# hendraet/synthesis-in-style

Hardware: AMD Instinct MI355X
Metric: StyleGAN2 synth images/sec + seg-train images/sec @256², 1/2/4/8 MI355X (higher is better)
Workload: dtype f32; 1 GPU; StyleGAN2 Generator(256,512,8,cm=2).forward, batch 32 per GPU, explicit noise, return_intermediate_activations=True (BASELINE.json configs[1]); batch_per_gpu=32, image_size=256, parallelism=replicated x1, images sharded, no collective

## Files before the change

### synthesis-in-style_amd/csrc/modconv_upfir.hip

```cpp
#include <type_traits>
#include "modconv_common.h"

namespace {

constexpr int UF_MBLK = 64;
constexpr int UF_PLANES = 16;
constexpr int UF_WROW = UF_PLANES * UF_MBLK + 32;
constexpr int UF_XP_MAX = 4;
constexpr unsigned UF_OOB = 0x80000000u;

struct UpFirParams {
    const float* x; const float* u; const float* s; const float* dscale; float* out;
    int B, Cin, Cout, H, W, OH, ORS;
    int nbw, bps, total_blocks;
    int vr;
    int rw4;
    int xs;
};

template <int PIPE, int ABL = 0, int NW = 8>
__global__ __launch_bounds__(64 * NW) __attribute__((amdgpu_waves_per_eu(2, 2))) void modconv_upfir_kernel(const UpFirParams p) {
    constexpr int UF_CC = NW, UF_NBLK = 8 * NW, UF_THREADS = 64 * NW;
    extern __shared__ __attribute__((aligned(16))) float lds[];
    float* Wl = lds;
    float* Xl = Wl + 2 * UF_CC * UF_WROW;
    float* Sl = Xl + 2 * UF_CC * p.xs;
    const int tid = threadIdx.x, lane = tid & 63, wave = __builtin_amdgcn_readfirstlane(tid >> 6);
    const int l15 = lane & 15, kq = lane >> 4;
    const int wm = wave & 1, wn = wave >> 1;

    const int n_co = p.Cout / UF_MBLK;
    const int tile = blockIdx.x / n_co, o0 = (blockIdx.x % n_co) * UF_MBLK;
    const int g0 = tile * UF_NBLK;
    const int b_first = g0 / p.bps, bh_first = (g0 % p.bps) / p.nbw;
    const int R0 = b_first * p.vr + 2 * bh_first;
    const int RW = 4 * p.rw4;
    const int HW = p.H * p.W;

    const int g = g0 + wn * 16 + l15;
    const bool live = g < p.total_blocks;
    const int gc = live ? g : p.total_blocks - 1;
    const int b = gc / p.bps, rem = gc % p.bps, bh = rem / p.nbw, bw = rem % p.nbw;
    const int xoff = (b * p.vr + 2 * bh - R0) * RW + 3 + 2 * bw;
    const int soff = (b - b_first) * p.Cin;

    for (int e = tid; e < 2 * p.Cin; e += UF_THREADS) {
        const int n = e / p.Cin, ci = e - n * p.Cin;
        Sl[e] = p.s[(int64_t)min(b_first + n, p.B - 1) * p.Cin + ci];
    }

    const __amdgpu_buffer_rsrc_t w_rsrc = sis_buffer_rsrc(p.u + 2 * o0);
    const __amdgpu_buffer_rsrc_t x_rsrc = sis_buffer_rsrc(p.x);
    const unsigned w_voff = (unsigned)(((lane >> 5) * p.Cout * 2 + (lane & 31) * 4) * 4);
    const int xpieces = p.xs >> 8;
    unsigned x_voff[UF_XP_MAX];
#pragma unroll
    for (int q = 0; q < UF_XP_MAX; ++q) {
        const int i = q * 64 + lane;
        const int row = i / p.rw4, c4 = i - row * p.rw4;
        const int v = R0 + row;
        const int bb = v / p.vr, h = v - bb * p.vr - 1, col = 4 * (c4 - 1);
        const bool ok = q < xpieces && bb < p.B && h >= 0 && h < p.H && col >= 0 && col < p.W;
        x_voff[q] = ok ? (unsigned)((bb * p.Cin * HW + h * p.W + col) * 4) : UF_OOB;
    }
    auto stage = [&](int ci0, int buf) {
        float* wdst = Wl + (buf * UF_CC + wave) * UF_WROW;
        const unsigned wbase = (unsigned)((ci0 + wave) * UF_PLANES * p.Cout * 4);
#pragma unroll
        for (int q = 0; q < 4; ++q) sis_buffer_load_lds16(w_rsrc, wdst + q * 256, w_voff, wbase + (unsigned)(q * 2 * p.Cout * 2 * 4));
        float* xdst = Xl + (buf * UF_CC + wave) * p.xs;
        const unsigned xbase = (unsigned)((ci0 + wave) * HW * 4);
#pragma unroll
        for (int q = 0; q < UF_XP_MAX; ++q)
            if (q < xpieces) sis_buffer_load_lds16(x_rsrc, xdst + q * 256, x_voff[q], xbase);
    };

    sis_f32x4 acc[5][5][2];
#pragma unroll
    for (int a = 0; a < 5; ++a)
#pragma unroll
        for (int c = 0; c < 5; ++c)
#pragma unroll
            for (int t = 0; t < 2; ++t) acc[a][c][t] = sis_f32x4{0.f, 0.f, 0.f, 0.f};

    __syncthreads();
    stage(0, 0);
    __syncthreads();

    if constexpr (PIPE == 4) {
        static_assert(NW == 4 && ABL == 0, "pipelined form: 4-wave workgroups, no ablations");
        const int n_chunks = p.Cin / UF_CC;
        if (n_chunks > 1) stage(UF_CC, 1);
        __syncthreads();
        float tA[4][4], tB[4][4], cm0[4], raw[3][3], svn;
        auto tr_read = [&](int c, int bufc) {
            const int cl = min(c, n_chunks - 1) * UF_CC + kq;
            svn = Sl[soff + cl];
            const float* xb = Xl + (bufc * UF_CC + kq) * p.xs + xoff;
#pragma unroll
            for (int r = 0; r < 3; ++r)
#pragma unroll
                for (int j = 0; j < 3; ++j) raw[r][j] = xb[r * RW + j];
        };
        auto tr_col = [&](int r, float (&t)[4][4]) {
            const float d0 = raw[r][0] * svn, d1 = raw[r][1] * svn, d2 = raw[r][2] * svn;
            float* o = r == 0 ? cm0 : (r == 1 ? t[1] : t[3]);
            o[0] = d0 - d1; o[1] = d1; o[2] = d2 - d1; o[3] = d2;
            asm volatile("" : "+v"(o[0]), "+v"(o[1]), "+v"(o[2]), "+v"(o[3]));
        };
        auto tr_row = [&](float (&t)[4][4]) {
#pragma unroll
            for (int j = 0; j < 4; ++j) {
                t[0][j] = cm0[j] - t[1][j]; t[2][j] = t[3][j] - t[1][j];
                asm volatile("" : "+v"(t[0][j]), "+v"(t[2][j]));
            }
        };
        tr_read(0, 0);
#pragma unroll
        for (int r = 0; r < 3; ++r) tr_col(r, tA);
        tr_row(tA);
        const int woff = kq * UF_WROW + (wm * 32 + l15) * 2;
        sis_f32x2 ra[3][2];
        ra[0][0] = *reinterpret_cast<const sis_f32x2*>(Wl + woff); ra[0][1] = *reinterpret_cast<const sis_f32x2*>(Wl + woff + 32);
        auto chunk = [&](auto parity, int c, const float (&t)[4][4], float (&tn)[4][4]) {
            constexpr int B = decltype(parity)::value;
            const float* wb = Wl + B * UF_CC * UF_WROW + woff;
            auto fetch = [&](int k) {
                ra[k % 3][0] = *reinterpret_cast<const sis_f32x2*>(wb + k * 2 * UF_MBLK);
                ra[k % 3][1] = *reinterpret_cast<const sis_f32x2*>(wb + k * 2 * UF_MBLK + 32);
            };
            fetch(1);
#pragma unroll
            for (int k = 0; k < 8; ++k) {
                if (k + 2 < 8) fetch(k + 2);
                if (k == 7) {
                    ra[0][0] = *reinterpret_cast<const sis_f32x2*>(Wl + (B ^ 1) * UF_CC * UF_WROW + woff);
                    ra[0][1] = *reinterpret_cast<const sis_f32x2*>(Wl + (B ^ 1) * UF_CC * UF_WROW + woff + 32);
                }
#pragma unroll
                for (int e = 0; e < 2; ++e) {
                    const int i = 2 * k + e, u = i >> 2, v = i & 3;
                    const float a0 = ra[k % 3][0][e], a1 = ra[k % 3][1][e];
#pragma unroll
                    for (int pp = 0; pp < 2; ++pp)
#pragma unroll
                        for (int qq = 0; qq < 2; ++qq) {
                            if ((pp && u != 3) || (qq && v != 3)) continue;
                            const int pi = u + pp, qi = v + qq;
                            const int di = pi == 3 ? 1 : (pi == 4 ? 3 : pi), dj = qi == 3 ? 1 : (qi == 4 ? 3 : qi);
                            acc[pi][qi][0] = __builtin_amdgcn_mfma_f32_16x16x4f32(a0, t[di][dj], acc[pi][qi][0], 0, 0, 0);
                            acc[pi][qi][1] = __builtin_amdgcn_mfma_f32_16x16x4f32(a1, t[di][dj], acc[pi][qi][1], 0, 0, 0);
                        }
                    if (k >= 5) {
                        if (k == 5 && e == 1) {
                            asm volatile("s_waitcnt vmcnt(0)" ::: "memory");
                            __syncthreads();
                            if (c + 2 < n_chunks) stage((c + 2) * UF_CC, B);
                            tr_read(c + 1, B ^ 1);
                        }
                        if (k == 6 && e == 0) { tr_col(0, tn); tr_col(1, tn); }
                        if (k == 6 && e == 1) tr_col(2, tn);
                        if (k == 7 && e == 0) tr_row(tn);
                        __builtin_amdgcn_sched_barrier(0);
                    }
                }
                if (k < 5) {
                    if (k + 2 < 8) __builtin_amdgcn_sched_group_barrier(0x100, 1, 0);
                    const int u = (2 * k) >> 2, vhi = ((2 * k) & 3) + 1;
                    if (u == 3 && vhi == 3) __builtin_amdgcn_sched_group_barrier(0x008, 12, 0);
                    else if (u == 3) __builtin_amdgcn_sched_group_barrier(0x008, 8, 0);
                    else if (vhi == 3) __builtin_amdgcn_sched_group_barrier(0x008, 6, 0);
                    else __builtin_amdgcn_sched_group_barrier(0x008, 4, 0);
                }
            }
        };
        for (int c = 0; c < n_chunks; c += 2) {
            chunk(std::integral_constant<int, 0>(), c, tA, tB);
            if (c + 1 < n_chunks) chunk(std::integral_constant<int, 1>(), c + 1, tB, tA);
        }
    } else {
    int buf = 0;
    float t0[4][4] = {}, t1[4][4] = {};
    const bool late_dma = PIPE == 3 && wave >= 4;
    for (int ci0 = 0; ci0 < p.Cin; ci0 += UF_CC, buf ^= 1) {
        if (!(ABL & 2) && !late_dma && ci0 + UF_CC < p.Cin) stage(ci0 + UF_CC, buf ^ 1);
        const float* Wb = Wl + buf * UF_CC * UF_WROW;
        const float* Xb = Xl + buf * UF_CC * p.xs;
        auto transform = [&](int ks, float (&t)[4][4]) {
            if constexpr (ABL & 4) {
                if (ci0 != 0) return;
            }
            const int cl = 4 * ks + kq;
            const float sv = Sl[soff + ci0 + cl];
            const float* xb = Xb + cl * p.xs + xoff;
            float c[3][4];
#pragma unroll
            for (int r = 0; r < 3; ++r) {
                const float d0 = xb[r * RW] * sv, d1 = xb[r * RW + 1] * sv, d2 = xb[r * RW + 2] * sv;
                c[r][0] = d0 - d1; c[r][1] = d1; c[r][2] = d2 - d1; c[r][3] = d2;
            }
#pragma unroll
            for (int j = 0; j < 4; ++j) {
                t[0][j] = c[0][j] - c[1][j]; t[1][j] = c[1][j]; t[2][j] = c[2][j] - c[1][j]; t[3][j] = c[2][j];
            }
        };
        auto multiply = [&](int ks, const float (&t)[4][4]) {
            const float* wb = Wb + (4 * ks + kq) * UF_WROW + (wm * 32 + l15) * 2;
            sis_f32x2 ra[3][2];
            auto fetch = [&](int k) {
                if constexpr (ABL & 8) {
                    ra[k % 3][0] = sis_f32x2{(float)(k + lane), (float)(k - lane)}; ra[k % 3][1] = sis_f32x2{(float)lane, (float)k};
                } else {
                    ra[k % 3][0] = *reinterpret_cast<const sis_f32x2*>(wb + k * 2 * UF_MBLK);
                    ra[k % 3][1] = *reinterpret_cast<const sis_f32x2*>(wb + k * 2 * UF_MBLK + 32);
                }
            };
            if constexpr (PIPE >= 1) { fetch(0); fetch(1); }
#pragma unroll
            for (int k = 0; k < 8; ++k) {
                if constexpr (PIPE >= 1) { if (k + 2 < 8) fetch(k + 2); }
                else fetch(k);
#pragma unroll
                for (int e = 0; e < 2; ++e) {
                    const int i = 2 * k + e, u = i >> 2, v = i & 3;
                    const float a0 = ra[k % 3][0][e], a1 = ra[k % 3][1][e];
#pragma unroll
                    for (int pp = 0; pp < 2; ++pp)
#pragma unroll
                        for (int qq = 0; qq < 2; ++qq) {
                            if ((pp && u != 3) || (qq && v != 3)) continue;
                            const int pi = u + pp, qi = v + qq;
                            const int di = pi == 3 ? 1 : (pi == 4 ? 3 : pi), dj = qi == 3 ? 1 : (qi == 4 ? 3 : qi);
                            acc[pi][qi][0] = __builtin_amdgcn_mfma_f32_16x16x4f32(a0, t[di][dj], acc[pi][qi][0], 0, 0, 0);
                            acc[pi][qi][1] = __builtin_amdgcn_mfma_f32_16x16x4f32(a1, t[di][dj], acc[pi][qi][1], 0, 0, 0);
                        }
                }
                if constexpr (PIPE >= 1) {
                    if (k + 2 < 8) __builtin_amdgcn_sched_group_barrier(0x100, 1, 0);
                    const int u = (2 * k) >> 2, vhi = ((2 * k) & 3) + 1;
                    if (u == 3 && vhi == 3) __builtin_amdgcn_sched_group_barrier(0x008, 12, 0);
                    else if (u == 3) __builtin_amdgcn_sched_group_barrier(0x008, 8, 0);
                    else if (vhi == 3) __builtin_amdgcn_sched_group_barrier(0x008, 6, 0);
                    else __builtin_amdgcn_sched_group_barrier(0x008, 4, 0);
                }
            }
        };
        if constexpr (NW == 4) {
            transform(0, t0);
            multiply(0, t0);
        } else if constexpr (PIPE == 2) {
            transform(0, t0);
            transform(1, t1);
            multiply(0, t0);
            multiply(1, t1);
        } else {
            transform(0, t0);
            multiply(0, t0);
            if (late_dma && ci0 + UF_CC < p.Cin) stage(ci0 + UF_CC, buf ^ 1);
            transform(1, t1);
            multiply(1, t1);
        }
        if constexpr (!(ABL & 1)) __syncthreads();
    }
    }

    int eg = g;
    if constexpr (PIPE == 4) { eg = g0 + wn * 16 + (int)(threadIdx.x & 15); asm volatile("" : "+v"(eg)); }
    if (eg >= p.total_blocks) return;
    int eb = b, ebh = bh, ebw = bw;
    if constexpr (PIPE == 4) { eb = eg / p.bps; const int erem = eg % p.bps; ebh = erem / p.nbw; ebw = erem % p.nbw; }
    const int OHW = p.OH * p.ORS;
    const float* db = p.dscale + (int64_t)eb * p.Cout;
    float* ob = p.out + (int64_t)eb * p.Cout * OHW + (int64_t)(4 * ebh) * p.ORS + 4 * ebw;
#pragma unroll
    for (int tt = 0; tt < 2; ++tt)
#pragma unroll
        for (int r = 0; r < 4; ++r) {
            const int co = o0 + wm * 32 + tt * 16 + 4 * kq + r;
            const float d = db[co];
            float cs[5][4];
#pragma unroll
            for (int pi = 0; pi < 5; ++pi) {
                cs[pi][0] = acc[pi][0][tt][r] + acc[pi][1][tt][r];
                cs[pi][1] = acc[pi][3][tt][r];
                cs[pi][2] = acc[pi][1][tt][r] + acc[pi][2][tt][r];
                cs[pi][3] = acc[pi][4][tt][r];
            }
            float* oc = ob + (int64_t)co * OHW;
#pragma unroll
            for (int ro = 0; ro < 4; ++ro) {
                float4 v;
                if (ro == 0) v = make_float4(cs[0][0] + cs[1][0], cs[0][1] + cs[1][1], cs[0][2] + cs[1][2], cs[0][3] + cs[1][3]);
                else if (ro == 1) v = make_float4(cs[3][0], cs[3][1], cs[3][2], cs[3][3]);
                else if (ro == 2) v = make_float4(cs[1][0] + cs[2][0], cs[1][1] + cs[2][1], cs[1][2] + cs[2][2], cs[1][3] + cs[2][3]);
                else v = make_float4(cs[4][0], cs[4][1], cs[4][2], cs[4][3]);
                *reinterpret_cast<float4*>(oc + ro * p.ORS) = make_float4(v.x * d, v.y * d, v.z * d, v.w * d);
            }
        }
}

#ifndef UF_EDGE_WAVES
#define UF_EDGE_WAVES 8
#endif
constexpr int UE_KC = 64;

template <bool ROWK, int NWV>
__device__ __forceinline__ void upfir_edge_tile(const UpFirParams& p, int tile, int cgb, float4* Dl) {
    constexpr int CSTEP = 4 * NWV, NR = UE_KC / CSTEP;
    const int tid = threadIdx.x, lane = tid & 63, wave = __builtin_amdgcn_readfirstlane(tid >> 6);
    const int l15 = lane & 15, kq = lane >> 4, sc = tid >> 4;
    const int co0 = (cgb * NWV + wave) * 16;
    const int per = ROWK ? p.W / 2 + 1 : p.H / 2;
    const int n_items = p.B * per;
    const int it = tile * 16 + l15;
    const int itc = it < n_items ? it : n_items - 1;
    const int b = itc / per, j = itc - b * per;
    const int HW = p.H * p.W;
    unsigned xo[3];
    bool ok[3];
#pragma unroll
    for (int r = 0; r < 3; ++r) {
        const int pos = 2 * j - 1 + r;
        ok[r] = pos >= 0 && pos < (ROWK ? p.W : p.H);
        xo[r] = (unsigned)(b * p.Cin * HW + (!ok[r] ? 0 : (ROWK ? (p.H - 1) * p.W + pos : pos * p.W + p.W - 1)));
    }
    const unsigned uo = (unsigned)(kq * UF_PLANES * p.Cout + (co0 + l15) * 2);

    float raw[NR][3], sv[NR];
    auto load_patch = [&](int c0) {
#pragma unroll
        for (int k = 0; k < NR; ++k) {
            const int ci = min(c0 + sc + k * CSTEP, p.Cin - 1);
            sv[k] = p.s[b * p.Cin + ci];
#pragma unroll
            for (int r = 0; r < 3; ++r) raw[k][r] = p.x[xo[r] + (unsigned)(ci * HW)];
        }
    };
    auto store_patch = [&](int buf) {
#pragma unroll
        for (int k = 0; k < NR; ++k) {
            Dl[(buf * UE_KC + sc + k * CSTEP) * 16 + l15] =
                make_float4(ok[0] ? raw[k][0] : 0.f, ok[1] ? raw[k][1] : 0.f, ok[2] ? raw[k][2] : 0.f, sv[k]);
        }
    };
    auto load_w = [&](int c0, float (&w)[16][4]) {
#pragma unroll
        for (int k = 0; k < 16; ++k) {
            const float* uc = p.u + (int64_t)min(c0 + 4 * k, p.Cin - 4) * UF_PLANES * p.Cout;
            if constexpr (ROWK) {
                const sis_f32x2 w0 = *reinterpret_cast<const sis_f32x2*>(uc + uo), w1 = *reinterpret_cast<const sis_f32x2*>(uc + 2 * p.Cout + uo);
                w[k][0] = w0[0]; w[k][1] = w0[1]; w[k][2] = w1[0]; w[k][3] = w1[1];
            } else {
#pragma unroll
                for (int u = 0; u < 4; ++u) w[k][u] = (uc + u * 4 * p.Cout)[uo];
            }
        }
    };

    sis_f32x4 acc[5];
#pragma unroll
    for (int a = 0; a < 5; ++a) acc[a] = sis_f32x4{0.f, 0.f, 0.f, 0.f};
    float wc[16][4], wn[16][4];
    load_patch(0);
    load_w(0, wc);
    store_patch(0);
    __syncthreads();
    for (int c0 = 0, buf = 0; c0 < p.Cin; c0 += UE_KC, buf ^= 1) {
        const bool more = c0 + UE_KC < p.Cin;
        if (more) { load_patch(c0 + UE_KC); load_w(c0 + UE_KC, wn); }
        const int ns = min(16, (p.Cin - c0) >> 2);
        auto step = [&](int k) {
            {
#pragma clang fp contract(off)
                const float4 dv = Dl[(buf * UE_KC + 4 * k + kq) * 16 + l15];
                const float sf = dv.w, z = sf * 0.f;
                float t[4];
                if constexpr (ROWK) {
                    const float d1 = sf * dv.y, d2 = sf * dv.z;
                    t[0] = __builtin_fmaf(sf, dv.x, -d1); t[1] = d1 - z; t[2] = __builtin_fmaf(sf, dv.z, -d1); t[3] = d2 - z;
                } else {
                    const float e0 = __builtin_fmaf(sf, dv.x, -z), e1 = __builtin_fmaf(sf, dv.y, -z), e2 = __builtin_fmaf(sf, dv.z, -z);
                    t[0] = e0 - e1; t[1] = e1; t[2] = e2 - e1; t[3] = e2;
                }
                acc[0] = __builtin_amdgcn_mfma_f32_16x16x4f32(wc[k][0], t[0], acc[0], 0, 0, 0);
                acc[1] = __builtin_amdgcn_mfma_f32_16x16x4f32(wc[k][1], t[1], acc[1], 0, 0, 0);
                acc[2] = __builtin_amdgcn_mfma_f32_16x16x4f32(wc[k][2], t[2], acc[2], 0, 0, 0);
                acc[3] = __builtin_amdgcn_mfma_f32_16x16x4f32(wc[k][3], t[1], acc[3], 0, 0, 0);
                acc[4] = __builtin_amdgcn_mfma_f32_16x16x4f32(wc[k][3], t[3], acc[4], 0, 0, 0);
            }
        };
        if (ns == 16) {
#pragma unroll
            for (int k = 0; k < 16; ++k) step(k);
        } else {
#pragma unroll
            for (int k = 0; k < 16; ++k)
                if (k < ns) step(k);
        }
        if (more) {
            store_patch(buf ^ 1);
#pragma unroll
            for (int k = 0; k < 16; ++k)
#pragma unroll
                for (int u = 0; u < 4; ++u) wc[k][u] = wn[k][u];
        }
        __syncthreads();
    }
    if (it >= n_items) return;
    const int OHW = p.OH * p.ORS;
#pragma unroll
    for (int r = 0; r < 4; ++r) {
        const int co = co0 + 4 * kq + r;
        const float dm = p.dscale[(int64_t)b * p.Cout + co];
        float* oc = p.out + ((int64_t)b * p.Cout + co) * OHW;
        if constexpr (ROWK) {
            const float v0 = (acc[0][r] + acc[1][r]) + 0.f, v1 = acc[3][r] + 0.f, v2 = (acc[1][r] + acc[2][r]) + 0.f, v3 = acc[4][r] + 0.f;
            *reinterpret_cast<float4*>(oc + (int64_t)(2 * p.H) * p.ORS + 4 * j) = make_float4(v0 * dm, v1 * dm, v2 * dm, v3 * dm);
        } else {
            const float c0 = acc[0][r] + 0.f, c1 = acc[1][r] + 0.f, c2 = acc[2][r] + 0.f, c3 = acc[3][r] + 0.f, c4 = acc[4][r] + 0.f;
            const float v[4] = {c0 + c1, c3, c1 + c2, c4};
            const float z = 0.f * dm;
#pragma unroll
            for (int ro = 0; ro < 4; ++ro)
                *reinterpret_cast<float4*>(oc + (int64_t)(4 * j + ro) * p.ORS + 2 * p.W) = make_float4(v[ro] * dm, z, z, z);
        }
    }
}

template <int NWV>
__global__ __launch_bounds__(64 * NWV) void modconv_upfir_edge_kernel(const UpFirParams p, int n_row_tiles) {
    __shared__ float4 Dl[2 * UE_KC * 16];
    const int n_cgb = p.Cout / (16 * NWV);
    const int tile = blockIdx.x / n_cgb, cgb = blockIdx.x - tile * n_cgb;
    if (tile < n_row_tiles) upfir_edge_tile<true, NWV>(p, tile, cgb, Dl);
    else upfir_edge_tile<false, NWV>(p, tile - n_row_tiles, cgb, Dl);
}

__global__ __launch_bounds__(256) void upfir_prepack_kernel(float* __restrict__ u, const float* __restrict__ w, int cout, int cin) {
    const int64_t i = (int64_t)blockIdx.x * 256 + threadIdx.x;
    if (i >= (int64_t)cout * cin) return;
    const int co = (int)(i % cout), ci = (int)(i / cout);
    const float* src = w + ((int64_t)co * cin + ci) * 9;
    float g[3][3];
#pragma unroll
    for (int t = 0; t < 9; ++t) g[t / 3][t % 3] = src[t];
    float rows[4][3];
#pragma unroll
    for (int kx = 0; kx < 3; ++kx) {
        rows[0][kx] = g[2][kx]; rows[1][kx] = g[0][kx] + g[2][kx]; rows[2][kx] = g[0][kx]; rows[3][kx] = g[1][kx];
    }
#pragma unroll
    for (int pu = 0; pu < 4; ++pu) {
        const float v4[4] = {rows[pu][2], rows[pu][0] + rows[pu][2], rows[pu][0], rows[pu][1]};
#pragma unroll
        for (int h = 0; h < 2; ++h)
            *reinterpret_cast<float2*>(u + (((int64_t)ci * 8 + pu * 2 + h) * cout + co) * 2) = make_float2(v4[2 * h], v4[2 * h + 1]);
    }
}

bool upfir_plan(UpFirParams& p, int batch, int cin, int cout, int h, int w, int row_stride, size_t* lds_bytes, int nw = 8) {
    const int UF_CC = nw, UF_NBLK = 8 * nw;
    static const int min_side = getenv("SIS_UPFIR_MIN_SIDE") ? atoi(getenv("SIS_UPFIR_MIN_SIDE")) : 16;
    if (batch <= 0 || h < min_side || w < min_side || (h & 1) || (w & 3) || cin % UF_CC || cout % UF_MBLK) return false;
    if ((row_stride & 3) || row_stride < 2 * w + 4) return false;
    if ((int64_t)batch * cin * h * w * 4 >= (1LL << 31) || (int64_t)cin * UF_PLANES * cout * 4 >= (1LL << 31)) return false;
    p.B = batch; p.Cin = cin; p.Cout = cout; p.H = h; p.W = w; p.OH = 2 * h + 1; p.ORS = row_stride;
    p.nbw = w / 2;
    const int nbh = h / 2;
    p.bps = nbh * p.nbw;
    if (p.bps < UF_NBLK) return false;
    p.total_blocks = batch * p.bps;
    p.vr = h + 1;
    p.rw4 = w / 4 + 2;
    const int n_tiles = sis_cdiv(p.total_blocks, UF_NBLK);
    int rows_max = 0;
    for (int t = 0; t < n_tiles; ++t) {
        const int g0 = t * UF_NBLK, g1 = (g0 + UF_NBLK - 1 < p.total_blocks ? g0 + UF_NBLK - 1 : p.total_blocks - 1);
        const int r0 = (g0 / p.bps) * p.vr + 2 * ((g0 % p.bps) / p.nbw);
        const int r1 = (g1 / p.bps) * p.vr + 2 * ((g1 % p.bps) / p.nbw) + 2;
        rows_max = r1 - r0 + 1 > rows_max ? r1 - r0 + 1 : rows_max;
    }
    p.xs = sis_cdiv(rows_max * 4 * p.rw4, 256) * 256;
    if (p.xs > 256 * UF_XP_MAX) return false;
    *lds_bytes = (size_t)(2 * UF_CC * UF_WROW + 2 * UF_CC * p.xs + 2 * cin) * sizeof(float);
    return *lds_bytes <= 160 * 1024;
}

}

static int upfir_waves() {
    static const int nw = getenv("SIS_UPFIR_WAVES") ? atoi(getenv("SIS_UPFIR_WAVES")) : 4;
    return nw;
}

extern "C" int sis_modconv_up_fir_supported(int batch, int cin, int cout, int h, int w, int t_row_stride) {
    UpFirParams p;
    size_t lds;
    const int nw = upfir_waves();
    return (nw == 4 || nw == 8) && upfir_plan(p, batch, cin, cout, h, w, t_row_stride, &lds, nw) ? 1 : 0;
}

extern "C" int sis_modconv_up_fir_prepack(float* u, const float* w, int cout, int cin, void* stream) {
    SIS_REQUIRE(u && w, "sis_modconv_up_fir_prepack: null pointer");
    SIS_REQUIRE(cout > 0 && cin > 0, "sis_modconv_up_fir_prepack: bad sizes");
    const int64_t n = (int64_t)cout * cin;
    hipLaunchKernelGGL(upfir_prepack_kernel, dim3(sis_cdiv(n, 256)), dim3(256), 0, (hipStream_t)stream, u, w, cout, cin);
    SIS_CHECK_LAUNCH("upfir_prepack_kernel");
    return 0;
}

extern "C" int sis_modconv2d_up_fir(float* t, const float* x, const float* u, const float* s, const float* dscale, int batch,
                                    int cin, int cout, int h, int w, int t_row_stride, void* stream) {
    if (batch == 0) return 0;
    SIS_REQUIRE(t && x && u && s && dscale, "sis_modconv2d_up_fir: null pointer");
    SIS_REQUIRE((((uintptr_t)t | (uintptr_t)x | (uintptr_t)u) & 15) == 0, "sis_modconv2d_up_fir: pointers must be 16-byte aligned");
    UpFirParams p;
    size_t lds;
    const int nw = upfir_waves();
    SIS_REQUIRE(nw == 4 || nw == 8, "sis_modconv2d_up_fir: SIS_UPFIR_WAVES must be 4 or 8");
    const int UF_NBLK = 8 * nw, UF_THREADS = 64 * nw;
    SIS_REQUIRE(upfir_plan(p, batch, cin, cout, h, w, t_row_stride, &lds, nw),
                "sis_modconv2d_up_fir: %d x (%d -> %d) on %d x %d with row stride %d is not supported (sis_modconv_up_fir_supported)", batch,
                cin, cout, h, w, t_row_stride);
    p.x = x; p.u = u; p.s = s; p.dscale = dscale; p.out = t;
    static bool attr_set = false;
    if (!attr_set) {
        hipError_t e = hipFuncSetAttribute(reinterpret_cast<const void*>(&modconv_upfir_kernel<0>), hipFuncAttributeMaxDynamicSharedMemorySize, 160 * 1024);
        if (e == hipSuccess) e = hipFuncSetAttribute(reinterpret_cast<const void*>(&modconv_upfir_kernel<1>), hipFuncAttributeMaxDynamicSharedMemorySize, 160 * 1024);
        if (e == hipSuccess) e = hipFuncSetAttribute(reinterpret_cast<const void*>(&modconv_upfir_kernel<2>), hipFuncAttributeMaxDynamicSharedMemorySize, 160 * 1024);
        if (e == hipSuccess) e = hipFuncSetAttribute(reinterpret_cast<const void*>(&modconv_upfir_kernel<3>), hipFuncAttributeMaxDynamicSharedMemorySize, 160 * 1024);
        if (e == hipSuccess) e = hipFuncSetAttribute(reinterpret_cast<const void*>(&modconv_upfir_kernel<1, 0, 4>), hipFuncAttributeMaxDynamicSharedMemorySize, 80 * 1024);
        if (e == hipSuccess) e = hipFuncSetAttribute(reinterpret_cast<const void*>(&modconv_upfir_kernel<0, 0, 4>), hipFuncAttributeMaxDynamicSharedMemorySize, 80 * 1024);
        if (e == hipSuccess) e = hipFuncSetAttribute(reinterpret_cast<const void*>(&modconv_upfir_kernel<4, 0, 4>), hipFuncAttributeMaxDynamicSharedMemorySize, 80 * 1024);
        if (e != hipSuccess) return sis_fail("sis_modconv2d_up_fir: cannot raise the dynamic LDS limit: %s", hipGetErrorString(e));
        attr_set = true;
    }
    const int64_t grid = (int64_t)sis_cdiv(p.total_blocks, UF_NBLK) * (cout / UF_MBLK);
    SIS_REQUIRE(grid > 0 && grid < ((int64_t)1 << 31), "sis_modconv2d_up_fir: bad grid");
    static const int pipe = getenv("SIS_UPFIR_PIPE") ? atoi(getenv("SIS_UPFIR_PIPE")) : 4;
#ifdef SIS_ABLATIONS
    static const int abl = getenv("SIS_UPFIR_ABL") ? atoi(getenv("SIS_UPFIR_ABL")) : 0;
    if (abl) {
        SIS_REQUIRE(nw == 8, "SIS_UPFIR_ABL: the ablations exist for SIS_UPFIR_WAVES=8 only");
#define UF_ABL(A) hipLaunchKernelGGL((modconv_upfir_kernel<1, A>), dim3((unsigned)grid), dim3(UF_THREADS), lds, (hipStream_t)stream, p)
        static bool abl_attr = false;
        if (!abl_attr) {
            (void)hipFuncSetAttribute(reinterpret_cast<const void*>(&modconv_upfir_kernel<1, 1>), hipFuncAttributeMaxDynamicSharedMemorySize, 160 * 1024);
            (void)hipFuncSetAttribute(reinterpret_cast<const void*>(&modconv_upfir_kernel<1, 2>), hipFuncAttributeMaxDynamicSharedMemorySize, 160 * 1024);
            (void)hipFuncSetAttribute(reinterpret_cast<const void*>(&modconv_upfir_kernel<1, 4>), hipFuncAttributeMaxDynamicSharedMemorySize, 160 * 1024);
            (void)hipFuncSetAttribute(reinterpret_cast<const void*>(&modconv_upfir_kernel<1, 8>), hipFuncAttributeMaxDynamicSharedMemorySize, 160 * 1024);
            (void)hipFuncSetAttribute(reinterpret_cast<const void*>(&modconv_upfir_kernel<1, 15>), hipFuncAttributeMaxDynamicSharedMemorySize, 160 * 1024);
            abl_attr = true;
        }
        if (abl == 1) UF_ABL(1); else if (abl == 2) UF_ABL(2); else if (abl == 4) UF_ABL(4); else if (abl == 8) UF_ABL(8); else UF_ABL(15);
#undef UF_ABL
        SIS_CHECK_LAUNCH("modconv_upfir_kernel<ablation>");
        sis_kernel_name = "modconv_upfir_kernel";
        return 0;
    }
#endif
    if (nw == 4 && pipe == 4) hipLaunchKernelGGL((modconv_upfir_kernel<4, 0, 4>), dim3((unsigned)grid), dim3(UF_THREADS), lds, (hipStream_t)stream, p);
    else if (nw == 4 && pipe == 0) hipLaunchKernelGGL((modconv_upfir_kernel<0, 0, 4>), dim3((unsigned)grid), dim3(UF_THREADS), lds, (hipStream_t)stream, p);
    else if (nw == 4) hipLaunchKernelGGL((modconv_upfir_kernel<1, 0, 4>), dim3((unsigned)grid), dim3(UF_THREADS), lds, (hipStream_t)stream, p);
    else if (pipe == 0) hipLaunchKernelGGL(modconv_upfir_kernel<0>, dim3((unsigned)grid), dim3(UF_THREADS), lds, (hipStream_t)stream, p);
    else if (pipe == 2) hipLaunchKernelGGL(modconv_upfir_kernel<2>, dim3((unsigned)grid), dim3(UF_THREADS), lds, (hipStream_t)stream, p);
    else if (pipe == 3) hipLaunchKernelGGL(modconv_upfir_kernel<3>, dim3((unsigned)grid), dim3(UF_THREADS), lds, (hipStream_t)stream, p);
    else hipLaunchKernelGGL(modconv_upfir_kernel<1>, dim3((unsigned)grid), dim3(UF_THREADS), lds, (hipStream_t)stream, p);
    SIS_CHECK_LAUNCH("modconv_upfir_kernel");
    const int n_row_tiles = sis_cdiv(batch * (w / 2 + 1), 16), n_tiles = n_row_tiles + sis_cdiv(batch * (h / 2), 16);
    if (cout % 128 == 0 && UF_EDGE_WAVES == 8) hipLaunchKernelGGL(modconv_upfir_edge_kernel<8>, dim3((unsigned)(n_tiles * (cout / 128))), dim3(512), 0, (hipStream_t)stream, p, n_row_tiles);
    else hipLaunchKernelGGL(modconv_upfir_edge_kernel<4>, dim3((unsigned)(n_tiles * (cout / 64))), dim3(256), 0, (hipStream_t)stream, p, n_row_tiles);
    SIS_CHECK_LAUNCH("modconv_upfir_edge_kernel");
    sis_kernel_name = "modconv_upfir_kernel";
    return 0;
}
```

Measured before the change: 2570 images/s.

## Stage upfir edge-kernel weights and inputs via async buffer-to-LDS ring

Rewrites the upfir edge kernel so weights and input edge strips are DMA'd straight into LDS through buffer_load_lds across a 3-deep ring of 8-channel chunks. The old path loaded them into registers and stored them to LDS, and kept 64 weight-register pairs in flight per thread. Style scales are staged once per tile into LDS. Row tiles now cover two 16-item strips so each staged weight chunk feeds twice as many MFMAs. The kernel switches to dynamic LDS and its LDS need is added to the eligibility check, which costs more LDS and adds complexity around vmcnt waits.

Result: no change. 2582 images/s, median of 6 (+0.5%).

```diff
diff --git a/synthesis-in-style_amd/csrc/modconv_upfir.hip b/synthesis-in-style_amd/csrc/modconv_upfir.hip
--- a/synthesis-in-style_amd/csrc/modconv_upfir.hip
+++ b/synthesis-in-style_amd/csrc/modconv_upfir.hip
@@ -302,138 +302,180 @@
 #ifndef UF_EDGE_WAVES
 #define UF_EDGE_WAVES 8
 #endif
-constexpr int UE_KC = 64;
-
-template <bool ROWK, int NWV>
-__device__ __forceinline__ void upfir_edge_tile(const UpFirParams& p, int tile, int cgb, float4* Dl) {
-    constexpr int CSTEP = 4 * NWV, NR = UE_KC / CSTEP;
+#ifndef UE_ROW_NS
+#define UE_ROW_NS 2
+#endif
+#ifndef UE_COL_NS
+#define UE_COL_NS 1
+#endif
+constexpr int UE_CC = 8;
+constexpr int UE_RING = 3;
+constexpr int ue_wrow(bool rowk, int nwv) { return (rowk ? 2 : 4) * 32 * nwv + 32; }
+constexpr int ue_xrow(int ns) { return 64 * ns + 17; }
+constexpr size_t ue_lds_floats(bool rowk, int nwv, int ns, int cin) {
+    return (size_t)UE_RING * UE_CC * (ue_wrow(rowk, nwv) + ue_xrow(ns)) + (size_t)(2 * ns + 1) * cin;
+}
+
+template <bool ROWK, int NWV, int NS>
+__device__ __forceinline__ void upfir_edge_tile(const UpFirParams& p, int tile, int cgb, float* lds) {
+    static_assert(NS == 1 || NS == 2, "a strip is NS DMA instructions of 64 entries");
+    constexpr int NP = ROWK ? 2 : 4;
+    constexpr int PF = 32 * NWV;
+    constexpr int WROW = ue_wrow(ROWK, NWV), XROW = ue_xrow(NS), NB = 16 * NS;
+    constexpr int LPP = 8 * NWV, PPI = 64 / LPP, NIW = NP / PPI;
+    constexpr int IPW = UE_CC * NIW / NWV, IPX = UE_CC * NS / NWV;
+    constexpr int ND = IPW + IPX;
+    static_assert(IPW % NIW == 0 && IPX % NS == 0, "a wave stages whole channels");
+    float* Wl = lds;
+    float* Xl = Wl + UE_RING * UE_CC * WROW;
+    float* Sl = Xl + UE_RING * UE_CC * XROW;
     const int tid = threadIdx.x, lane = tid & 63, wave = __builtin_amdgcn_readfirstlane(tid >> 6);
-    const int l15 = lane & 15, kq = lane >> 4, sc = tid >> 4;
-    const int co0 = (cgb * NWV + wave) * 16;
+    const int l15 = lane & 15, kq = lane >> 4;
+    const int o0 = cgb * 16 * NWV;
     const int per = ROWK ? p.W / 2 + 1 : p.H / 2;
+    const int lim = ROWK ? p.W : p.H;
     const int n_items = p.B * per;
-    const int it = tile * 16 + l15;
-    const int itc = it < n_items ? it : n_items - 1;
-    const int b = itc / per, j = itc - b * per;
+    const int it0 = tile * NB, b0 = it0 / per;
+    const int last = min(it0 + NB, n_items) - 1;
+    const int e_max = 2 * (last - it0) + 2 * (last / per - b0) + 2;
     const int HW = p.H * p.W;
-    unsigned xo[3];
-    bool ok[3];
-#pragma unroll
-    for (int r = 0; r < 3; ++r) {
-        const int pos = 2 * j - 1 + r;
-        ok[r] = pos >= 0 && pos < (ROWK ? p.W : p.H);
-        xo[r] = (unsigned)(b * p.Cin * HW + (!ok[r] ? 0 : (ROWK ? (p.H - 1) * p.W + pos : pos * p.W + p.W - 1)));
-    }
-    const unsigned uo = (unsigned)(kq * UF_PLANES * p.Cout + (co0 + l15) * 2);
-
-    float raw[NR][3], sv[NR];
-    auto load_patch = [&](int c0) {
-#pragma unroll
-        for (int k = 0; k < NR; ++k) {
-            const int ci = min(c0 + sc + k * CSTEP, p.Cin - 1);
-            sv[k] = p.s[b * p.Cin + ci];
-#pragma unroll
-            for (int r = 0; r < 3; ++r) raw[k][r] = p.x[xo[r] + (unsigned)(ci * HW)];
+    const int n_chunks = (p.Cin + UE_CC - 1) / UE_CC;
+
+    for (int e = tid; e < (2 * NS + 1) * p.Cin; e += 64 * NWV) {
+        const int n = e / p.Cin, ci = e - n * p.Cin;
+        Sl[e] = p.s[(int64_t)min(b0 + n, p.B - 1) * p.Cin + ci];
+    }
+
+    const __amdgpu_buffer_rsrc_t w_rsrc = sis_buffer_rsrc(p.u + 2 * o0);
+    const __amdgpu_buffer_rsrc_t x_rsrc = sis_buffer_rsrc(p.x);
+    const unsigned pstride = (unsigned)((ROWK ? 1 : 2) * p.Cout * 2 * 4);
+    const unsigned w_voff = (unsigned)(lane / LPP) * pstride + (unsigned)(lane % LPP) * 16u;
+    unsigned x_voff[NS];
+#pragma unroll
+    for (int h = 0; h < NS; ++h) {
+        const int e = h * 64 + lane, a = e + 2 * (it0 + b0);
+        const int b = a / (2 * (per + 1)), pos = a - b * 2 * (per + 1) - 1;
+        const bool ok = e <= e_max && pos >= 0 && pos < lim;
+        x_voff[h] = ok ? (unsigned)((b * p.Cin * HW + (ROWK ? (p.H - 1) * p.W + pos : pos * p.W + p.W - 1)) * 4) : UF_OOB;
+    }
+    auto stage = [&](int c, int rb) {
+#pragma unroll
+        for (int t = 0; t < IPW; ++t) {
+            const int ch = wave * (IPW / NIW) + t / NIW, q = t % NIW, ci = c * UE_CC + ch;
+            sis_buffer_load_lds16(w_rsrc, Wl + (rb * UE_CC + ch) * WROW + q * PPI * PF, ci < p.Cin ? w_voff : UF_OOB,
+                                  (unsigned)(min(ci, p.Cin - 1) * UF_PLANES * p.Cout * 4) + (unsigned)(q * PPI) * pstride);
+        }
+#pragma unroll
+        for (int t = 0; t < IPX; ++t) {
+            const int ch = wave * (IPX / NS) + t / NS, h = t % NS, ci = c * UE_CC + ch;
+            __builtin_amdgcn_raw_ptr_buffer_load_lds(x_rsrc, (sis_lds_void*)(Xl + (rb * UE_CC + ch) * XROW + h * 64), 4,
+                                                     ci < p.Cin ? x_voff[h] : UF_OOB, (unsigned)(min(ci, p.Cin - 1) * HW * 4), 0, 0);
         }
     };
-    auto store_patch = [&](int buf) {
-#pragma unroll
-        for (int k = 0; k < NR; ++k) {
-            Dl[(buf * UE_KC + sc + k * CSTEP) * 16 + l15] =
-                make_float4(ok[0] ? raw[k][0] : 0.f, ok[1] ? raw[k][1] : 0.f, ok[2] ? raw[k][2] : 0.f, sv[k]);
-        }
-    };
-    auto load_w = [&](int c0, float (&w)[16][4]) {
-#pragma unroll
-        for (int k = 0; k < 16; ++k) {
-            const float* uc = p.u + (int64_t)min(c0 + 4 * k, p.Cin - 4) * UF_PLANES * p.Cout;
+
+    int eo[NS], so[NS];
+#pragma unroll
+    for (int n = 0; n < NS; ++n) {
+        const int itc = min(it0 + n * 16 + l15, n_items - 1), b = itc / per;
+        eo[n] = 2 * (itc - it0) + 2 * (b - b0);
+        so[n] = (b - b0) * p.Cin;
+    }
+
+    sis_f32x4 acc[NS][5];
+#pragma unroll
+    for (int n = 0; n < NS; ++n)
+#pragma unroll
+        for (int a = 0; a < 5; ++a) acc[n][a] = sis_f32x4{0.f, 0.f, 0.f, 0.f};
+
+    __syncthreads();
+    stage(0, 0);
+    if (n_chunks > 1) stage(1, 1);
+    const int woff = kq * WROW + (wave * 16 + l15) * 2;
+    for (int c = 0, rb = 0, rn = 2; c < n_chunks; ++c) {
+        if (c + 1 < n_chunks) asm volatile("s_waitcnt vmcnt(%0)" ::"n"(ND) : "memory");
+        else asm volatile("s_waitcnt vmcnt(0)" ::: "memory");
+        __builtin_amdgcn_s_barrier();
+        if (c + 2 < n_chunks) stage(c + 2, rn);
+        const float* Wb = Wl + rb * UE_CC * WROW + woff;
+        const float* Xb = Xl + (rb * UE_CC + kq) * XROW;
+        auto step = [&](int k) {
+            const int ci = c * UE_CC + 4 * k + kq;
+            {
+                const float* wb = Wb + 4 * k * WROW;
+                float w[4];
+                if constexpr (ROWK) {
+                    const sis_f32x2 w0 = *reinterpret_cast<const sis_f32x2*>(wb), w1 = *reinterpret_cast<const sis_f32x2*>(wb + PF);
+                    w[0] = w0[0]; w[1] = w0[1]; w[2] = w1[0]; w[3] = w1[1];
+                } else {
+#pragma unroll
+                    for (int u = 0; u < 4; ++u) w[u] = wb[u * PF];
+                }
+#pragma unroll
+                for (int n = 0; n < NS; ++n) {
+#pragma clang fp contract(off)
+                    const float* xb = Xb + 4 * k * XROW + eo[n];
+                    const float x0 = xb[0], x1 = xb[1], x2 = xb[2];
+                    const float sf = Sl[so[n] + min(ci, p.Cin - 1)], z = sf * 0.f;
+                    float t[4];
+                    if constexpr (ROWK) {
+                        const float d1 = sf * x1, d2 = sf * x2;
+                        t[0] = __builtin_fmaf(sf, x0, -d1); t[1] = d1 - z; t[2] = __builtin_fmaf(sf, x2, -d1); t[3] = d2 - z;
+                    } else {
+                        const float e0 = __builtin_fmaf(sf, x0, -z), e1 = __builtin_fmaf(sf, x1, -z), e2 = __builtin_fmaf(sf, x2, -z);
+                        t[0] = e0 - e1; t[1] = e1; t[2] = e2 - e1; t[3] = e2;
+                    }
+                    acc[n][0] = __builtin_amdgcn_mfma_f32_16x16x4f32(w[0], t[0], acc[n][0], 0, 0, 0);
+                    acc[n][1] = __builtin_amdgcn_mfma_f32_16x16x4f32(w[1], t[1], acc[n][1], 0, 0, 0);
+                    acc[n][2] = __builtin_amdgcn_mfma_f32_16x16x4f32(w[2], t[2], acc[n][2], 0, 0, 0);
+                    acc[n][3] = __builtin_amdgcn_mfma_f32_16x16x4f32(w[3], t[1], acc[n][3], 0, 0, 0);
+                    acc[n][4] = __builtin_amdgcn_mfma_f32_16x16x4f32(w[3], t[3], acc[n][4], 0, 0, 0);
+                }
+            }
+        };
+#pragma unroll
+        for (int k = 0; k < UE_CC / 4; ++k) step(k);
+        rb = rb == UE_RING - 1 ? 0 : rb + 1;
+        rn = rn == UE_RING - 1 ? 0 : rn + 1;
+    }
+
+    const int OHW = p.OH * p.ORS;
+#pragma unroll
+    for (int n = 0; n < NS; ++n) {
+        const int it = it0 + n * 16 + l15;
+        if (it >= n_items) continue;
+        const int b = it / per, j = it - b * per;
+#pragma unroll
+        for (int r = 0; r < 4; ++r) {
+            const int co = o0 + wave * 16 + 4 * kq + r;
+            const float dm = p.dscale[(int64_t)b * p.Cout + co];
+            float* oc = p.out + ((int64_t)b * p.Cout + co) * OHW;
             if constexpr (ROWK) {
-                const sis_f32x2 w0 = *reinterpret_cast<const sis_f32x2*>(uc + uo), w1 = *reinterpret_cast<const sis_f32x2*>(uc + 2 * p.Cout + uo);
-                w[k][0] = w0[0]; w[k][1] = w0[1]; w[k][2] = w1[0]; w[k][3] = w1[1];
+                const float v0 = (acc[n][0][r] + acc[n][1][r]) + 0.f, v1 = acc[n][3][r] + 0.f, v2 = (acc[n][1][r] + acc[n][2][r]) + 0.f, v3 = acc[n][4][r] + 0.f;
+                *reinterpret_cast<float4*>(oc + (int64_t)(2 * p.H) * p.ORS + 4 * j) = make_float4(v0 * dm, v1 * dm, v2 * dm, v3 * dm);
             } else {
-#pragma unroll
-                for (int u = 0; u < 4; ++u) w[k][u] = (uc + u * 4 * p.Cout)[uo];
-            }
-        }
-    };
-
-    sis_f32x4 acc[5];
-#pragma unroll
-    for (int a = 0; a < 5; ++a) acc[a] = sis_f32x4{0.f, 0.f, 0.f, 0.f};
-    float wc[16][4], wn[16][4];
-    load_patch(0);
-    load_w(0, wc);
-    store_patch(0);
-    __syncthreads();
-    for (int c0 = 0, buf = 0; c0 < p.Cin; c0 += UE_KC, buf ^= 1) {
-        const bool more = c0 + UE_KC < p.Cin;
-        if (more) { load_patch(c0 + UE_KC); load_w(c0 + UE_KC, wn); }
-        const int ns = min(16, (p.Cin - c0) >> 2);
-        auto step = [&](int k) {
-            {
-#pragma clang fp contract(off)
-                const float4 dv = Dl[(buf * UE_KC + 4 * k + kq) * 16 + l15];
-                const float sf = dv.w, z = sf * 0.f;
-                float t[4];
-                if constexpr (ROWK) {
-                    const float d1 = sf * dv.y, d2 = sf * dv.z;
-                    t[0] = __builtin_fmaf(sf, dv.x, -d1); t[1] = d1 - z; t[2] = __builtin_fmaf(sf, dv.z, -d1); t[3] = d2 - z;
-                } else {
-                    const float e0 = __builtin_fmaf(sf, dv.x, -z), e1 = __builtin_fmaf(sf, dv.y, -z), e2 = __builtin_fmaf(sf, dv.z, -z);
-                    t[0] = e0 - e1; t[1] = e1; t[2] = e2 - e1; t[3] = e2;
-                }
-                acc[0] = __builtin_amdgcn_mfma_f32_16x16x4f32(wc[k][0], t[0], acc[0], 0, 0, 0);
-                acc[1] = __builtin_amdgcn_mfma_f32_16x16x4f32(wc[k][1], t[1], acc[1], 0, 0, 0);
-                acc[2] = __builtin_amdgcn_mfma_f32_16x16x4f32(wc[k][2], t[2], acc[2], 0, 0, 0);
-                acc[3] = __builtin_amdgcn_mfma_f32_16x16x4f32(wc[k][3], t[1], acc[3], 0, 0, 0);
-                acc[4] = __builtin_amdgcn_mfma_f32_16x16x4f32(wc[k][3], t[3], acc[4], 0, 0, 0);
-            }
-        };
-        if (ns == 16) {
-#pragma unroll
-            for (int k = 0; k < 16; ++k) step(k);
-        } else {
-#pragma unroll
-            for (int k = 0; k < 16; ++k)
-                if (k < ns) step(k);
-        }
-        if (more) {
-            store_patch(buf ^ 1);
-#pragma unroll
-            for (int k = 0; k < 16; ++k)
-#pragma unroll
-                for (int u = 0; u < 4; ++u) wc[k][u] = wn[k][u];
-        }
-        __syncthreads();
-    }
-    if (it >= n_items) return;
-    const int OHW = p.OH * p.ORS;
-#pragma unroll
-    for (int r = 0; r < 4; ++r) {
-        const int co = co0 + 4 * kq + r;
-        const float dm = p.dscale[(int64_t)b * p.Cout + co];
-        float* oc = p.out + ((int64_t)b * p.Cout + co) * OHW;
-        if constexpr (ROWK) {
-            const float v0 = (acc[0][r] + acc[1][r]) + 0.f, v1 = acc[3][r] + 0.f, v2 = (acc[1][r] + acc[2][r]) + 0.f, v3 = acc[4][r] + 0.f;
-            *reinterpret_cast<float4*>(oc + (int64_t)(2 * p.H) * p.ORS + 4 * j) = make_float4(v0 * dm, v1 * dm, v2 * dm, v3 * dm);
-        } else {
-            const float c0 = acc[0][r] + 0.f, c1 = acc[1][r] + 0.f, c2 = acc[2][r] + 0.f, c3 = acc[3][r] + 0.f, c4 = acc[4][r] + 0.f;
-            const float v[4] = {c0 + c1, c3, c1 + c2, c4};
-            const float z = 0.f * dm;
-#pragma unroll
-            for (int ro = 0; ro < 4; ++ro)
-                *reinterpret_cast<float4*>(oc + (int64_t)(4 * j + ro) * p.ORS + 2 * p.W) = make_float4(v[ro] * dm, z, z, z);
+                const float c0 = acc[n][0][r] + 0.f, c1 = acc[n][1][r] + 0.f, c2 = acc[n][2][r] + 0.f, c3 = acc[n][3][r] + 0.f, c4 = acc[n][4][r] + 0.f;
+                const float v[4] = {c0 + c1, c3, c1 + c2, c4};
+                const float z = 0.f * dm;
+#pragma unroll
+                for (int ro = 0; ro < 4; ++ro)
+                    *reinterpret_cast<float4*>(oc + (int64_t)(4 * j + ro) * p.ORS + 2 * p.W) = make_float4(v[ro] * dm, z, z, z);
+            }
         }
     }
 }
 
 template <int NWV>
 __global__ __launch_bounds__(64 * NWV) void modconv_upfir_edge_kernel(const UpFirParams p, int n_row_tiles) {
-    __shared__ float4 Dl[2 * UE_KC * 16];
+    extern __shared__ __attribute__((aligned(16))) float lds[];
     const int n_cgb = p.Cout / (16 * NWV);
     const int tile = blockIdx.x / n_cgb, cgb = blockIdx.x - tile * n_cgb;
-    if (tile < n_row_tiles) upfir_edge_tile<true, NWV>(p, tile, cgb, Dl);
-    else upfir_edge_tile<false, NWV>(p, tile - n_row_tiles, cgb, Dl);
+    if (tile < n_row_tiles) upfir_edge_tile<true, NWV, UE_ROW_NS>(p, tile, cgb, lds);
+    else upfir_edge_tile<false, NWV, UE_COL_NS>(p, tile - n_row_tiles, cgb, lds);
+}
+
+size_t upfir_edge_lds(int cin, int nwv) {
+    const size_t r = ue_lds_floats(true, nwv, UE_ROW_NS, cin), c = ue_lds_floats(false, nwv, UE_COL_NS, cin);
+    return (r > c ? r : c) * sizeof(float);
 }
 
 __global__ __launch_bounds__(256) void upfir_prepack_kernel(float* __restrict__ u, const float* __restrict__ w, int cout, int cin) {
@@ -462,6 +504,7 @@
     const int UF_CC = nw, UF_NBLK = 8 * nw;
     static const int min_side = getenv("SIS_UPFIR_MIN_SIDE") ? atoi(getenv("SIS_UPFIR_MIN_SIDE")) : 16;
     if (batch <= 0 || h < min_side || w < min_side || (h & 1) || (w & 3) || cin % UF_CC || cout % UF_MBLK) return false;
+    if (h < 16 || w < 16) return false;
     if ((row_stride & 3) || row_stride < 2 * w + 4) return false;
     if ((int64_t)batch * cin * h * w * 4 >= (1LL << 31) || (int64_t)cin * UF_PLANES * cout * 4 >= (1LL << 31)) return false;
     p.B = batch; p.Cin = cin; p.Cout = cout; p.H = h; p.W = w; p.OH = 2 * h + 1; p.ORS = row_stride;
@@ -483,7 +526,7 @@
     p.xs = sis_cdiv(rows_max * 4 * p.rw4, 256) * 256;
     if (p.xs > 256 * UF_XP_MAX) return false;
     *lds_bytes = (size_t)(2 * UF_CC * UF_WROW + 2 * UF_CC * p.xs + 2 * cin) * sizeof(float);
-    return *lds_bytes <= 160 * 1024;
+    return *lds_bytes <= 160 * 1024 && upfir_edge_lds(cin, cout % 128 == 0 && UF_EDGE_WAVES == 8 ? 8 : 4) <= 160 * 1024;
 }
 
 }
@@ -532,6 +575,8 @@
         if (e == hipSuccess) e = hipFuncSetAttribute(reinterpret_cast<const void*>(&modconv_upfir_kernel<1, 0, 4>), hipFuncAttributeMaxDynamicSharedMemorySize, 80 * 1024);
         if (e == hipSuccess) e = hipFuncSetAttribute(reinterpret_cast<const void*>(&modconv_upfir_kernel<0, 0, 4>), hipFuncAttributeMaxDynamicSharedMemorySize, 80 * 1024);
         if (e == hipSuccess) e = hipFuncSetAttribute(reinterpret_cast<const void*>(&modconv_upfir_kernel<4, 0, 4>), hipFuncAttributeMaxDynamicSharedMemorySize, 80 * 1024);
+        if (e == hipSuccess) e = hipFuncSetAttribute(reinterpret_cast<const void*>(&modconv_upfir_edge_kernel<8>), hipFuncAttributeMaxDynamicSharedMemorySize, 160 * 1024);
+        if (e == hipSuccess) e = hipFuncSetAttribute(reinterpret_cast<const void*>(&modconv_upfir_edge_kernel<4>), hipFuncAttributeMaxDynamicSharedMemorySize, 160 * 1024);
         if (e != hipSuccess) return sis_fail("sis_modconv2d_up_fir: cannot raise the dynamic LDS limit: %s", hipGetErrorString(e));
         attr_set = true;
     }
@@ -567,9 +612,9 @@
     else if (pipe == 3) hipLaunchKernelGGL(modconv_upfir_kernel<3>, dim3((unsigned)grid), dim3(UF_THREADS), lds, (hipStream_t)stream, p);
     else hipLaunchKernelGGL(modconv_upfir_kernel<1>, dim3((unsigned)grid), dim3(UF_THREADS), lds, (hipStream_t)stream, p);
     SIS_CHECK_LAUNCH("modconv_upfir_kernel");
-    const int n_row_tiles = sis_cdiv(batch * (w / 2 + 1), 16), n_tiles = n_row_tiles + sis_cdiv(batch * (h / 2), 16);
-    if (cout % 128 == 0 && UF_EDGE_WAVES == 8) hipLaunchKernelGGL(modconv_upfir_edge_kernel<8>, dim3((unsigned)(n_tiles * (cout / 128))), dim3(512), 0, (hipStream_t)stream, p, n_row_tiles);
-    else hipLaunchKernelGGL(modconv_upfir_edge_kernel<4>, dim3((unsigned)(n_tiles * (cout / 64))), dim3(256), 0, (hipStream_t)stream, p, n_row_tiles);
+    const int n_row_tiles = sis_cdiv(batch * (w / 2 + 1), 16 * UE_ROW_NS), n_tiles = n_row_tiles + sis_cdiv(batch * (h / 2), 16 * UE_COL_NS);
+    if (cout % 128 == 0 && UF_EDGE_WAVES == 8) hipLaunchKernelGGL(modconv_upfir_edge_kernel<8>, dim3((unsigned)(n_tiles * (cout / 128))), dim3(512), upfir_edge_lds(cin, 8), (hipStream_t)stream, p, n_row_tiles);
+    else hipLaunchKernelGGL(modconv_upfir_edge_kernel<4>, dim3((unsigned)(n_tiles * (cout / 64))), dim3(256), upfir_edge_lds(cin, 4), (hipStream_t)stream, p, n_row_tiles);
     SIS_CHECK_LAUNCH("modconv_upfir_edge_kernel");
     sis_kernel_name = "modconv_upfir_kernel";
     return 0;
```
